# zju3dv/DetectorFreeSfM

Measured on NVIDIA B200. Metric: image-pairs/s coarse-match (hp2: tracks/s refinement), higher is better.
Workload: dtype f16x2-split (fp32-grade), fp32 accumulate

## Files before the change

### detectorfreesfm_b200/_lib.py

```python
import ctypes
import os

_HERE = os.path.dirname(os.path.abspath(__file__))
LIB_PATH = os.path.join(_HERE, "libdfsfm_b200.so")

_lib = None

c_void_p, c_int, c_float, c_char_p, c_int64 = ctypes.c_void_p, ctypes.c_int, ctypes.c_float, ctypes.c_char_p, ctypes.c_int64

PROTOTYPES = {
    "dfsfm_last_error": (c_char_p, []),
    "dfsfm_version": (c_int, []),
    "dfsfm_launch_count": (c_int64, []),
    "dfsfm_thread_set_pdl": (None, [c_int]),
    "dfsfm_debug_gemm_slab": (c_int, [c_void_p, c_int64, c_int, c_void_p, c_int64, c_int, c_void_p, c_int, c_int, c_int, c_void_p,
                                      c_int, c_int, c_void_p]),
    "dfsfm_set_engine": (None, [c_int]),
    "dfsfm_get_engine": (c_int, []),
    "dfsfm_profile_enable": (None, [c_int]),
    "dfsfm_profile_report": (c_int, [c_char_p, c_int]),
    "dfsfm_post_create": (c_int, [ctypes.POINTER(c_void_p), c_int]),
    "dfsfm_post_destroy": (None, [c_void_p]),
    "dfsfm_post_merge_keypoints": (c_int, [c_void_p, c_void_p, c_int64, c_int, c_void_p, c_void_p, c_int, c_void_p, c_void_p, c_void_p, c_void_p,
                                           ctypes.POINTER(c_int64), c_void_p]),
    "dfsfm_resize_lanczos_gray": (c_int, [c_void_p, c_int, c_int, c_int64, c_void_p, c_void_p, c_int, c_void_p, c_void_p, c_int, c_int, c_int,
                                          c_void_p, c_void_p, c_void_p]),
    "dfsfm_debug_timeline_arm": (c_int, [c_int]),
    "dfsfm_debug_timeline_read": (c_int, [c_void_p, c_void_p, c_int]),
    "dfsfm_coarse_create": (c_int, [ctypes.POINTER(c_void_p), c_int]),
    "dfsfm_coarse_destroy": (None, [c_void_p]),
    "dfsfm_coarse_set_param": (c_int, [c_void_p, c_char_p, c_void_p, c_int64, c_int64, c_int]),
    "dfsfm_coarse_features": (c_int, [c_void_p, c_void_p, c_int, c_int, c_void_p, c_void_p, c_void_p]),
    "dfsfm_coarse_features_fine": (c_int, [c_void_p, c_void_p, c_int, c_int, c_void_p, c_void_p, c_void_p, c_void_p]),
    "dfsfm_coarse_fine_match": (c_int, [c_void_p, c_void_p, c_int, c_int, c_void_p, c_int, c_int, c_void_p, c_int, c_void_p, c_int, c_void_p,
                                        c_void_p, c_int, c_void_p, c_void_p, c_void_p]),
    "dfsfm_coarse_transformer": (c_int, [c_void_p, c_void_p, c_int, c_void_p, c_int, c_void_p]),
    "dfsfm_coarse_match": (c_int, [c_void_p, c_void_p, c_int, c_int, c_void_p, c_int, c_int, c_float, c_int, c_float,
                                   c_void_p, c_void_p, c_void_p, c_void_p, c_int, c_void_p, c_void_p]),
    "dfsfm_crop_and_resize_forward": (c_int, [c_void_p, c_int, c_int, c_int, c_int, c_void_p, c_void_p, c_int, c_float,
                                              c_int, c_int, c_void_p, c_void_p]),
    "dfsfm_refine_create": (c_int, [ctypes.POINTER(c_void_p), c_int, c_int, c_int]),
    "dfsfm_refine_destroy": (None, [c_void_p]),
    "dfsfm_refine_set_param": (c_int, [c_void_p, c_char_p, c_void_p, c_int64, c_int64, c_int]),
    "dfsfm_refine_chunk": (c_int, [c_void_p, c_int, c_void_p, c_void_p, c_void_p, c_void_p, c_int, c_int, c_void_p, c_void_p,
                                   c_void_p, c_void_p, c_void_p, c_void_p, c_void_p, c_void_p, c_void_p, c_void_p]),
    "dfsfm_assign_bags": (c_int, [ctypes.POINTER(c_void_p), c_int64, c_void_p, c_void_p, c_void_p, c_void_p, c_int64, c_void_p, c_void_p, c_void_p,
                                  c_int, c_int, c_int]),
    "dfsfm_bags_sizes": (None, [c_void_p, ctypes.POINTER(c_int64), ctypes.POINTER(c_int64), ctypes.POINTER(c_int64), ctypes.POINTER(c_int64)]),
    "dfsfm_bags_export": (None, [c_void_p, c_void_p, c_void_p, c_void_p, c_void_p, c_void_p, c_void_p, c_void_p]),
    "dfsfm_bags_destroy": (None, [c_void_p]),
    "dfsfm_debug_pyset": (c_int, [c_int, c_void_p, c_int64, c_void_p, c_int64, c_void_p, ctypes.POINTER(c_int64)]),
    "dfsfm_debug_gemm": (c_int, [c_void_p, c_int64, c_int, c_void_p, c_int64, c_int, c_void_p, c_int, c_int, c_int, c_void_p,
                                 c_int, c_int, c_void_p]),
}


class DfsfmError(RuntimeError):
    pass


def load_library():
    global _lib
    if _lib is not None:
        return _lib
    if not os.path.exists(LIB_PATH):
# ... 25 lines not shown
```

### detectorfreesfm_b200/coarse_matcher.py

```python
import ctypes
from collections import OrderedDict

import torch

from . import _lib
from .packing import pack_loftr, position_encoding


class B200LoFTR(torch.nn.Module):
    def __init__(self, config, device=None, feature_cache_size=64, feature_cache_bytes=8 << 30):
        super().__init__()
        self.config = config
        mc = config["match_coarse"]
        if mc["match_type"] != "dual_softmax":
            raise NotImplementedError("only match_type='dual_softmax' is built (the shipped loftr_ds configs)")
        self.fine = bool(config["fine"]["enable"])
        if self.fine:
            fcfg = config["fine"]
            if (fcfg["d_model"] != 128 or fcfg["nhead"] != 8 or list(fcfg["layer_names"]) != ["self", "cross"] or config["fine_window_size"] != 5
                    or not config["fine_concat_coarse_feat"] or tuple(config["resolution"]) != (8, 2)):
                raise NotImplementedError("fine stage is specialised for the outdoor_ds LoFTR (window 5, d_model 128, ['self','cross'])")
        c = config["coarse"]
        if c["d_model"] != 256 or c["nhead"] != 8 or list(c["layer_names"]) != ["self", "cross"] * 4 or c["attention"] != "linear":
            raise NotImplementedError("engine is specialised for the outdoor_ds LoFTR (d_model 256, 8 heads, 8 layers, linear)")
# ... 32 lines not shown
        return self

    def load_state_dict(self, state_dict, strict=True):
        self._packed = pack_loftr(state_dict, fine=self.fine)
        if self._h:
            self._upload()
        self.clear_cache()
        return self

    def _upload(self):
        for name, (t, kind) in self._packed.items():
            _lib.check(self._lib.dfsfm_coarse_set_param(self._h, name.encode(), ctypes.c_void_p(t.data_ptr()), t.shape[0], t.shape[1], kind))

    def _destroy(self):
        if self._h:
            self._lib.dfsfm_coarse_destroy(self._h)
            self._h = ctypes.c_void_p()
        self._pe.clear()
        self._cache.clear()
        self._cache_bytes = 0

    def __del__(self):
        try:
            self._destroy()
        except Exception:
            pass

    def _pe_tokens(self, h, w):
        key = (h, w)
        if key not in self._pe:
            self._pe[key] = position_encoding(h, w).to(self._device)
        return self._pe[key]

    def extract_features(self, image, cache_key=None):
        assert image.is_cuda and image.dtype == torch.float32 and image.dim() == 4 and image.shape[0] == 1 and image.shape[1] == 1
        H, W = image.shape[2:]
        key = None if cache_key is None else (cache_key, H, W)
        if key is not None and key in self._cache:
            self._cache.move_to_end(key)
            return self._cache[key]
        image = image.contiguous()
        h, w = H // 8, W // 8
        tokens = torch.empty(h * w, 256, device=self._device, dtype=torch.float32)
        if self.fine:
            feat_f = torch.empty((H // 2) * (W // 2), 128, device=self._device, dtype=torch.float32)
            _lib.check(self._lib.dfsfm_coarse_features_fine(self._h, _lib.ptr(image), H, W, _lib.ptr(self._pe_tokens(h, w)), _lib.ptr(tokens),
                                                            _lib.ptr(feat_f), _lib.stream_ptr(self._device)))
            out = (tokens, feat_f)
        else:
            _lib.check(self._lib.dfsfm_coarse_features(self._h, _lib.ptr(image), H, W, _lib.ptr(self._pe_tokens(h, w)), _lib.ptr(tokens),
                                                       _lib.stream_ptr(self._device)))
            out = tokens
        if key is not None:
            nbytes = sum(t.numel() * t.element_size() for t in (out if isinstance(out, tuple) else (out,)))
            self._cache[key] = out
            self._cache_bytes += nbytes
            while len(self._cache) > 1 and (len(self._cache) > self._cache_size or self._cache_bytes > self._cache_bytes_max):
                _, old = self._cache.popitem(last=False)
                self._cache_bytes -= sum(t.numel() * t.element_size() for t in (old if isinstance(old, tuple) else (old,)))
        return out

    def fine_match(self, feat_f0, hw0_f, feat_f1, hw1_f, feat_c0, hw0_c, feat_c1, hw1_c, i_ids, j_ids):
        M = int(i_ids.shape[0])
        coords = torch.zeros(M, 2, device=self._device, dtype=torch.float32)
        std = torch.zeros(M, device=self._device, dtype=torch.float32)
        if M > 0:
            i32, j32 = i_ids.to(torch.int32).contiguous(), j_ids.to(torch.int32).contiguous()
            _lib.check(self._lib.dfsfm_coarse_fine_match(self._h, _lib.ptr(feat_f0), hw0_f[0], hw0_f[1], _lib.ptr(feat_f1), hw1_f[0], hw1_f[1],
                                                         _lib.ptr(feat_c0), hw0_c[1], _lib.ptr(feat_c1), hw1_c[1], _lib.ptr(i32), _lib.ptr(j32), M,
                                                         _lib.ptr(coords), _lib.ptr(std), _lib.stream_ptr(self._device)))
        return coords, std

    def transform(self, feat0, feat1):
        _lib.check(self._lib.dfsfm_coarse_transformer(self._h, _lib.ptr(feat0), feat0.shape[0], _lib.ptr(feat1), feat1.shape[0],
                                                      _lib.stream_ptr(self._device)))
        return feat0, feat1

    def coarse_match(self, feat0, hw0_c, feat1, hw1_c, return_conf=False):
        L, S = hw0_c[0] * hw0_c[1], hw1_c[0] * hw1_c[1]
        cap = min(L, S)
        i_ids = torch.empty(cap, device=self._device, dtype=torch.int32)
        j_ids = torch.empty(cap, device=self._device, dtype=torch.int32)
        mconf = torch.empty(cap, device=self._device, dtype=torch.float32)
        count = torch.zeros(1, device=self._device, dtype=torch.int32)
        conf = torch.empty(L, S, device=self._device, dtype=torch.float32) if return_conf else None
        _lib.check(self._lib.dfsfm_coarse_match(self._h, _lib.ptr(feat0), hw0_c[0], hw0_c[1], _lib.ptr(feat1), hw1_c[0], hw1_c[1],
                                                self.thr, self.border_rm, self.temperature, _lib.ptr(i_ids), _lib.ptr(j_ids),
                                                _lib.ptr(mconf), _lib.ptr(count), cap, _lib.ptr(conf), _lib.stream_ptr(self._device)))
        n = int(count.item())
        return i_ids[:n].long(), j_ids[:n].long(), mconf[:n], conf

    @torch.no_grad()
    def forward(self, data):
        if not self._h:
            raise _lib.DfsfmError("B200LoFTR: call .cuda() before forward (there is no CPU path)")
        with torch.cuda.device(self._device):
            return self._forward(data)

    def clear_cache(self):
        self._cache.clear()
        self._cache_bytes = 0

    def _forward(self, data):
        if not self._h:
            raise _lib.DfsfmError("B200LoFTR: call .cuda() before forward (there is no CPU path)")
        if self._packed is None:
            raise _lib.DfsfmError("B200LoFTR: load_state_dict() has not been called")
        im0, im1 = data["image0"], data["image1"]
        if im0.size(0) != 1:
            raise NotImplementedError("bs must be 1 (coarse_match_worker.py:86 asserts the same)")
        if "mask0" in data:
            raise NotImplementedError("padding masks are a training-time feature (loftr.py:61-63)")
        data.update({"bs": 1, "hw0_i": im0.shape[2:], "hw1_i": im1.shape[2:]})
        names = data.get("pair_key")
        k0 = k1 = None
        if names is not None:
            k0 = names[0][0] if isinstance(names[0], (list, tuple)) else names[0]
            k1 = names[1][0] if isinstance(names[1], (list, tuple)) else names[1]
        f0 = self.extract_features(im0, k0)
        f1 = self.extract_features(im1, k1)
        if self.fine:
            (f0, ff0), (f1, ff1) = f0, f1
        hw0_c = (im0.shape[2] // 8, im0.shape[3] // 8)
        hw1_c = (im1.shape[2] // 8, im1.shape[3] // 8)
        data.update({"hw0_c": torch.Size(hw0_c), "hw1_c": torch.Size(hw1_c)})
        f0, f1 = self.transform(f0.clone(), f1.clone())
        keep_conf = bool(data.get("_return_conf_matrix", False))
        i_ids, j_ids, mconf, conf = self.coarse_match(f0, hw0_c, f1, hw1_c, keep_conf)
        if keep_conf:
            data["conf_matrix"] = conf[None]
            data["feat_c0"], data["feat_c1"] = f0[None], f1[None]
        b_ids = torch.zeros_like(i_ids)
        scale = data["hw0_i"][0] / hw0_c[0]
        scale0 = scale * data["scale0"][b_ids][:, [1, 0]] if "scale0" in data else scale
        scale1 = scale * data["scale1"][b_ids][:, [1, 0]] if "scale1" in data else scale
        mkpts0_c = torch.stack([i_ids % hw0_c[1], i_ids // hw0_c[1]], dim=1) * scale0
        mkpts1_c = torch.stack([j_ids % hw1_c[1], j_ids // hw1_c[1]], dim=1) * scale1
        keep = mconf != 0
        data.update({
            "b_ids": b_ids, "i_ids": i_ids, "j_ids": j_ids, "gt_mask": mconf == 0,
            "m_bids": b_ids[keep], "mkpts0_c": mkpts0_c[keep], "mkpts1_c": mkpts1_c[keep], "mconf": mconf[keep],
        })
        if not self.fine:
            data.update({"mkpts0_f": data["mkpts0_c"], "mkpts1_f": data["mkpts1_c"]})
            return None
        hw0_f = (im0.shape[2] // 2, im0.shape[3] // 2)
        hw1_f = (im1.shape[2] // 2, im1.shape[3] // 2)
        data.update({"hw0_f": torch.Size(hw0_f), "hw1_f": torch.Size(hw1_f), "W": 5})
        coords2, std = self.fine_match(ff0, hw0_f, ff1, hw1_f, f0, hw0_c, f1, hw1_c, i_ids, j_ids)
        data["expec_f"] = torch.cat([coords2 / 2, std[:, None]], -1)
        scale_f = data["hw0_i"][0] / hw0_f[0]
        scale1_f = scale_f * data["scale1"][b_ids][:, [1, 0]] if "scale0" in data else scale_f
        data.update({"mkpts0_f": data["mkpts0_c"], "mkpts1_f": data["mkpts1_c"] + (coords2 * scale1_f)[:len(data["mconf"])]})
# ... 2 lines not shown
```

### detectorfreesfm_b200/csrc/coarse_engine.cu

```cuda
#include <algorithm>
#include <map>
#include <memory>

#include "../../include/dfsfm_b200.h"
#include "engine_common.h"
#include "fine_kernels.cuh"
#include "refine_kernels.cuh"

namespace dfsfm {

namespace {

struct Geom {
    int H, W, Hp, Wp;
    long long rows;
    Geom() : H(0), W(0), Hp(0), Wp(0), rows(0) {}
    Geom(int h, int w) : H(h), W(w), Hp(h + 1), Wp(w + 1), rows(static_cast<long long>(h + 1) * (w + 1)) {}
    FlatGeom flat() const { return FlatGeom{Hp, Wp, H, W}; }
};

struct ParityBuf {
    __half* base = nullptr;
    long long rows = 0;
    int C = 0;
    HL plane(int k) const {
        HL b;
        b.hi = base + static_cast<long long>(k) * 2 * rows * C;
        b.rows = rows;
        b.C = C;
        return b;
    }
    long long plane_stride() const { return 2 * rows * C; }
};

struct FeatWs {
// ... 19 lines not shown
struct TokWs {
    int cap = 0;
    HL x[2], msg[2], m1[2], hid[2];
    float* qkv[2] = {nullptr, nullptr};
    float* xf = nullptr;
    HL g;
    float* ksum = nullptr;
    float* kvp_part = nullptr;
    unsigned* kvp_flags = nullptr;
    int L = 0, L1 = 0, S = 0;
    int kv_chunks = 0;
    float* kv_part = nullptr;
    float* kv_state = nullptr;
    Seg* seg_dev = nullptr;
    float2* part = nullptr;
    float* stat[2] = {nullptr, nullptr};
    unsigned long long* best[2] = {nullptr, nullptr};
};

}

class CoarseEngine {
  public:
    explicit CoarseEngine(int device) : device_(device) {
        DFSFM_CUDA(cudaSetDevice(device));
        DFSFM_CUDA(cudaFuncSetAttribute(attn_apply_kernel<32>, cudaFuncAttributeMaxDynamicSharedMemorySize, attn_smem_bytes<32>()));
    }
    ~CoarseEngine() {
        for (auto& kv : feat_ws_) free_feat(kv.second);
        free_tok(tok_);
    }
    ParamStore params;

    void features(const float* img, int H, int W, const float* pe, float* tokens, float* feat_f, cudaStream_t st);
    void fine_match(const float* ff0, int Hf0, int Wf0, const float* ff1, int Hf1, int Wf1, const float* fc0, int w0c, const float* fc1, int w1c,
                    const int* i_ids, const int* j_ids, int M, float* coords_out, float* std_out, cudaStream_t st);
    void transformer(float* f0, int L, float* f1, int S, cudaStream_t st);
    void match(const float* f0, int h0c, int w0c, const float* f1, int h1c, int w1c, float thr, int border, float temperature, int* i_ids,
               int* j_ids, float* mconf, int* n_matches, int capacity, float* conf_out, cudaStream_t st);

  private:
    int device_;
    std::map<std::pair<int, int>, FeatWs> feat_ws_;
    TokWs tok_;
    unsigned kv_epoch_ = 0;
    FineWs fine_;
    void ensure_fine(int M);
    void fine_branch(FeatWs& w, float* feat_f, cudaStream_t st);
    void layer128(int li, bool self, int x0, int xn, int s0, int sn, const Seg* kv_segs, int n_kv, const Seg* apply_segs, int n_apply, cudaStream_t st);

    FeatWs& get_feat_ws(int H, int W);
    void ensure_tok(int n);
    static void free_feat(FeatWs& w);
    static void free_tok(TokWs& w);

    template <int BN>
    void conv(const HL* ins, int n_in, GemmCore core, const std::string& wname, ConvEpiParams ep, cudaStream_t st);
    void layer_call(int li, bool self, int x0, int xn, int s0, int sn, int kv_seg0, int n_segs, int apply_seg0, int max_count, cudaStream_t st,
                    int seg_row0 = 0);
};

static int kv_tok() {
    static int v = 0;
    if (!v) {
        const char* e = getenv("DFSFM_KV_TOK");
        v = e ? atoi(e) : kKvTokPerCta;
        if (v < 16) v = 16;
    }
    return v;
}
static bool attn_fold() {
    static int v = -1;
    if (v < 0) {
        const char* e = getenv("DFSFM_ATTN_FOLD");
        v = (e && e[0] == '0') ? 0 : 1;
    }
    return v == 1 && engine_version() == 2;
}
static bool kv_epi() {
    static int v = -1;
    if (v < 0) {
        const char* e = getenv("DFSFM_KV_EPI");
        v = (e && e[0] == '0') ? 0 : 1;
    }
    return v == 1;
}
static bool enc_fused() {
    static int v = -1;
    if (v < 0) {
        const char* e = getenv("DFSFM_ENC_FUSED");
        v = (e && e[0] == '0') ? 0 : 1;
    }
    return v == 1;
}
static bool lin_bn128() {
    static int v = -1;
    if (v < 0) {
        const char* e = getenv("DFSFM_LIN_BN128");
        v = (e && e[0] == '1') ? 1 : 0;
    }
    return v == 1;
}

static ParityBuf parity_alloc(long long rows, int C) {
    ParityBuf p;
    p.rows = rows;
    p.C = C;
    const size_t bytes = static_cast<size_t>(8) * rows * C * sizeof(__half);
    DFSFM_CUDA(cudaMalloc(&p.base, bytes));
    zero_device_sync(p.base, 0, bytes);
    return p;
}

FeatWs& CoarseEngine::get_feat_ws(int H, int W) {
    auto key = std::make_pair(H, W);
    auto it = feat_ws_.find(key);
    if (it != feat_ws_.end()) return it->second;
    if (feat_ws_.size() >= 8) {
        for (auto& kv : feat_ws_) free_feat(kv.second);
        feat_ws_.clear();
    }
    FeatWs w;
    w.g2 = Geom(H / 2, W / 2);
    w.g4 = Geom(H / 4, W / 4);
    w.g8 = Geom(H / 8, W / 8);
    w.a2 = hl_alloc(w.g2.rows, 128);
    w.b2 = hl_alloc(w.g2.rows, 128);
    w.c2 = hl_alloc(w.g2.rows, 128);
    w.p1 = parity_alloc(w.g4.rows, 128);
    w.a4 = hl_alloc(w.g4.rows, 208);
    w.b4 = hl_alloc(w.g4.rows, 208);
    w.p2 = parity_alloc(w.g8.rows, 208);
    w.a8 = hl_alloc(w.g8.rows, 256);
    w.b8 = hl_alloc(w.g8.rows, 256);
    w.c8 = hl_alloc(w.g8.rows, 256);
    return feat_ws_.emplace(key, w).first->second;
}
void CoarseEngine::free_feat(FeatWs& w) {
    hl_free(w.a2); hl_free(w.b2); hl_free(w.c2); hl_free(w.a4); hl_free(w.b4); hl_free(w.a8); hl_free(w.b8); hl_free(w.c8);
    if (w.p1.base) cudaFree(w.p1.base);
    if (w.p2.base) cudaFree(w.p2.base);
    if (w.fine) {
        hl_free(w.x3o); hl_free(w.t4a); hl_free(w.t4b); hl_free(w.x2o); hl_free(w.t2a); hl_free(w.t2b);
        cudaFree(w.f4); cudaFree(w.f2);
    }
}

template <int BN>
void CoarseEngine::conv(const HL* ins, int n_in, GemmCore core, const std::string& wname, ConvEpiParams ep, cudaStream_t st) {
    const HL& w = params.mat(wname + ".w");
    const bool slab = BN <= 128 && slab_applicable(core, n_in);
    TmapPack maps;
    for (int i = 0; i < kMaxAMaps; ++i) maps.a[i] = make_tmap(ins[i < n_in ? i : 0], slab ? kSlabRows : kBM);
    maps.b = make_tmap(w, bbox(BN));
    core.b_row0 = 0;
    DFSFM_CHECK(static_cast<long long>(core.num_taps) * core.cpad == w.C, "weight K does not match taps*cpad for " + wname);
    ep.M = core.M;
    ep.bias = params.has_vec(wname + ".b") ? params.vec(wname + ".b") : nullptr;
    if constexpr (BN <= 128) {
        if (slab) {
            launch_gemm_slab_counted<BN, ConvEpi>(maps, core, ep, ep.N, st, "conv");
            return;
        }
    }
    launch_gemm_counted<BN, true, ConvEpi>(maps, core, ep, ep.N, st, "conv");
}

static ConvEpiParams epi_flat(const Geom& g, int N, const HL& out, bool relu, const HL* res) {
    ConvEpiParams e;
    memset(&e, 0, sizeof(e));
    e.N = N;
    e.g = g.flat();
    e.relu = relu ? 1 : 0;
    if (res) { e.res_hi = res->hi; e.res_lo = res->lo(); e.res_ld = res->C; }
    e.out_mode = OUT_FLAT;
    e.out_hi = out.hi;
    e.out_lo = out.lo();
    e.out_ld = out.C;
    return e;
}
static ConvEpiParams epi_parity(const Geom& g, int N, const ParityBuf& out, bool relu, const HL* res) {
    ConvEpiParams e = epi_flat(g, N, out.plane(0), relu, res);
    e.out_mode = OUT_PARITY;
    e.plane_stride = out.plane_stride();
    return e;
}

void CoarseEngine::features(const float* img, int H, int W, const float* pe, float* tokens, float* feat_f, cudaStream_t st) {
    DFSFM_CHECK(H % 8 == 0 && W % 8 == 0 && H >= 16 && W >= 16, "image size must be a multiple of 8 (CoarseMatchingDataset df=8)");
    FeatWs& w = get_feat_ws(H, W);
    {
        dim3 grid((w.g2.W + kStemTW - 1) / kStemTW, (w.g2.H + kStemTH - 1) / kStemTH, 1);
        { LaunchScope ls("stem", st);
          stem_conv_kernel<<<grid, 128, 0, st>>>(img, H, W, params.vec("stem.w"), params.vec("stem.b"), w.a2.hi, w.a2.lo()); }
        DFSFM_CUDA(cudaGetLastError());
    }
    GemmCore c;
    memset(&c, 0, sizeof(c));
    c.M = static_cast<int>(w.g2.rows);
    set_k(c, 128);
    conv_taps_s1(c, 3, w.g2.Wp);
    { const HL in[1] = {w.a2}; conv<128>(in, 1, c, "l1.0.c1", epi_flat(w.g2, 128, w.b2, true, nullptr), st); }
    { const HL in[1] = {w.b2}; conv<128>(in, 1, c, "l1.0.c2", epi_flat(w.g2, 128, w.c2, true, &w.a2), st); }
    { const HL in[1] = {w.c2}; conv<128>(in, 1, c, "l1.1.c1", epi_flat(w.g2, 128, w.b2, true, nullptr), st); }
    { const HL in[1] = {w.b2}; conv<128>(in, 1, c, "l1.1.c2", epi_parity(w.g2, 128, w.p1, true, &w.c2), st); }
    c.M = static_cast<int>(w.g4.rows);
    set_k(c, 128);
    conv_taps_s2(c, w.g4.Wp);
    { const HL in[4] = {w.p1.plane(0), w.p1.plane(1), w.p1.plane(2), w.p1.plane(3)};
      conv<208>(in, 4, c, "l2.0.c1", epi_flat(w.g4, 208, w.a4, true, nullptr), st); }
    set_k(c, 208);
    conv_taps_s1(c, 3, w.g4.Wp);
    c.num_taps = 10; c.tap_map[9] = 1; c.tap_shift[9] = 0;
    { const HL in[2] = {w.a4, w.p1.plane(0)}; conv<208>(in, 2, c, "l2.0.c2", epi_flat(w.g4, 208, w.b4, true, nullptr), st); }
    conv_taps_s1(c, 3, w.g4.Wp);
    { const HL in[1] = {w.b4}; conv<208>(in, 1, c, "l2.1.c1", epi_flat(w.g4, 208, w.a4, true, nullptr), st); }
    { const HL in[1] = {w.a4}; conv<208>(in, 1, c, "l2.1.c2", epi_parity(w.g4, 208, w.p2, true, &w.b4), st); }
    c.M = static_cast<int>(w.g8.rows);
    set_k(c, 208);
    conv_taps_s2(c, w.g8.Wp);
    { const HL in[4] = {w.p2.plane(0), w.p2.plane(1), w.p2.plane(2), w.p2.plane(3)};
      conv<256>(in, 4, c, "l3.0.c1", epi_flat(w.g8, 256, w.a8, true, nullptr), st); }
    set_k(c, 256);
    conv_taps_s1(c, 3, w.g8.Wp);
    c.num_taps = 10; c.tap_map[9] = 1; c.tap_shift[9] = 0;
    { const HL in[2] = {w.a8, w.p2.plane(0)}; conv<256>(in, 2, c, "l3.0.c2", epi_flat(w.g8, 256, w.b8, true, nullptr), st); }
    conv_taps_s1(c, 3, w.g8.Wp);
    { const HL in[1] = {w.b8}; conv<256>(in, 1, c, "l3.1.c1", epi_flat(w.g8, 256, w.a8, true, nullptr), st); }
    { const HL in[1] = {w.a8}; conv<256>(in, 1, c, "l3.1.c2", epi_flat(w.g8, 256, w.c8, true, &w.b8), st); }
    conv_taps_s1(c, 1, w.g8.Wp);
    {
        ConvEpiParams e;
        memset(&e, 0, sizeof(e));
        e.N = 256;
        e.g = w.g8.flat();
        e.addend = pe;
        e.out_mode = OUT_DENSE;
        e.out_f32 = tokens;
        e.out_f32_ld = 256;
        if (feat_f) {
            if (!w.fine) {
                w.x3o = hl_alloc(w.g8.rows, 256);
                w.t4a = hl_alloc(w.g4.rows, 256); w.t4b = hl_alloc(w.g4.rows, 256); w.x2o = hl_alloc(w.g4.rows, 208);
                w.t2a = hl_alloc(w.g2.rows, 208); w.t2b = hl_alloc(w.g2.rows, 208);
                DFSFM_CUDA(cudaMalloc(&w.f4, static_cast<size_t>(w.g4.rows) * 256 * sizeof(float)));
                DFSFM_CUDA(cudaMalloc(&w.f2, static_cast<size_t>(w.g2.rows) * 208 * sizeof(float)));
                w.fine = true;
            }
        }
        const HL in[1] = {w.c8};
        conv<256>(in, 1, c, "out3", e, st);
        if (feat_f) {
            ConvEpiParams e2 = epi_flat(w.g8, 256, w.x3o, false, nullptr);
            conv<256>(in, 1, c, "out3", e2, st);
            fine_branch(w, feat_f, st);
        }
    }
}

void CoarseEngine::fine_branch(FeatWs& w, float* feat_f, cudaStream_t st) {
    GemmCore c;
    memset(&c, 0, sizeof(c));
    auto up_add = [&](const HL& low, const Geom& gl, int C, const float* lateral, const HL& out) {
        const long long total = static_cast<long long>(2 * gl.H) * (2 * gl.W) * (C / 8);
        LaunchScope ls("upsample", st);
        upsample2x_add_kernel<<<static_cast<unsigned>((total + 255) / 256), 256, 0, st>>>(low.hi, low.lo(), gl.H, gl.W, C, lateral, out.hi, out.lo(), total);
        DFSFM_CUDA(cudaGetLastError());
    };
    c.M = static_cast<int>(w.g8.rows);
    set_k(c, 208);
    conv_taps_s1(c, 1, w.g8.Wp);
    for (int k = 0; k < 4; ++k) {
        ConvEpiParams e;
        memset(&e, 0, sizeof(e));
        e.N = 256; e.g = w.g8.flat(); e.out_mode = OUT_UNPARITY; e.upy = k >> 1; e.upx = k & 1; e.ohp = w.g4.Hp; e.owp = w.g4.Wp;
        e.out_f32 = w.f4; e.out_f32_ld = 256;
        const HL in[1] = {w.p2.plane(k)};
        conv<256>(in, 1, c, "fpn.l2o", e, st);
    }
    up_add(w.x3o, w.g8, 256, w.f4, w.t4a);
    c.M = static_cast<int>(w.g4.rows);
    set_k(c, 256);
    conv_taps_s1(c, 3, w.g4.Wp);
    { ConvEpiParams e = epi_flat(w.g4, 256, w.t4b, false, nullptr); e.relu = 2; const HL in[1] = {w.t4a}; conv<256>(in, 1, c, "fpn.l2o2a", e, st); }
    { ConvEpiParams e = epi_flat(w.g4, 208, w.x2o, false, nullptr); const HL in[1] = {w.t4b}; conv<208>(in, 1, c, "fpn.l2o2b", e, st); }
    set_k(c, 128);
    conv_taps_s1(c, 1, w.g4.Wp);
// ... 516 lines not shown
    }
    layer128(0, true, 0, R, 0, R, f.segs, 2 * M, f.segs, 2 * M, st);
    layer128(1, false, 0, MW, MW, MW, f.segs + M, M, f.segs + 2 * M, M, st);
    layer128(1, false, MW, MW, 0, MW, f.segs, M, f.segs + 3 * M, M, st);
    {
        const size_t smem = fine_match_smem_bytes(5, 1);
        DFSFM_CUDA(cudaMemsetAsync(coords_out, 0, static_cast<size_t>(M) * 2 * sizeof(float), st));
        LaunchScope ls("fine_match", st);
        fine_match_kernel<<<M, kFmThreads, smem, st>>>(f.xf, f.tracks, f.views, 1, 5, 1, f.d_query, coords_out, std_out, M);
        DFSFM_CUDA(cudaGetLastError());
    }
}

}

using dfsfm::CoarseEngine;
struct dfsfm_coarse { std::unique_ptr<CoarseEngine> e; };

extern "C" {

int dfsfm_coarse_create(dfsfm_coarse_t** out, int device) {
    return dfsfm::guard([&] {
        auto* h = new dfsfm_coarse;
        h->e.reset(new CoarseEngine(device));
        *out = h;
    });
}
void dfsfm_coarse_destroy(dfsfm_coarse_t* h) { delete h; }

int dfsfm_coarse_set_param(dfsfm_coarse_t* h, const char* name, const float* host, int64_t rows, int64_t cols, int kind) {
    return dfsfm::guard([&] { h->e->params.set(name, host, rows, cols, kind); });
}
int dfsfm_coarse_features(dfsfm_coarse_t* h, const float* image_dev, int H, int W, const float* pe_dev, float* tokens_out_dev, void* stream) {
    return dfsfm::guard([&] { h->e->features(image_dev, H, W, pe_dev, tokens_out_dev, nullptr, static_cast<cudaStream_t>(stream)); });
}
int dfsfm_coarse_features_fine(dfsfm_coarse_t* h, const float* image_dev, int H, int W, const float* pe_dev, float* tokens_out_dev,
                               float* feat_f_out_dev, void* stream) {
    return dfsfm::guard([&] { h->e->features(image_dev, H, W, pe_dev, tokens_out_dev, feat_f_out_dev, static_cast<cudaStream_t>(stream)); });
}
int dfsfm_coarse_fine_match(dfsfm_coarse_t* h, const float* feat_f0_dev, int Hf0, int Wf0, const float* feat_f1_dev, int Hf1, int Wf1,
                            const float* feat_c0_dev, int w0c, const float* feat_c1_dev, int w1c, const int32_t* i_ids_dev,
                            const int32_t* j_ids_dev, int M, float* coords_out_dev, float* std_out_dev, void* stream) {
    return dfsfm::guard([&] {
        h->e->fine_match(feat_f0_dev, Hf0, Wf0, feat_f1_dev, Hf1, Wf1, feat_c0_dev, w0c, feat_c1_dev, w1c, i_ids_dev, j_ids_dev, M, coords_out_dev,
                         std_out_dev, static_cast<cudaStream_t>(stream));
    });
}
int dfsfm_coarse_transformer(dfsfm_coarse_t* h, float* feat0_dev, int L, float* feat1_dev, int S, void* stream) {
    return dfsfm::guard([&] { h->e->transformer(feat0_dev, L, feat1_dev, S, static_cast<cudaStream_t>(stream)); });
}
int dfsfm_coarse_match(dfsfm_coarse_t* h, const float* feat0_dev, int h0c, int w0c, const float* feat1_dev, int h1c, int w1c, float thr,
                       int border_rm, float temperature, int32_t* i_ids_dev, int32_t* j_ids_dev, float* mconf_dev, int32_t* n_matches_dev,
                       int capacity, float* conf_out_dev, void* stream) {
    return dfsfm::guard([&] {
        h->e->match(feat0_dev, h0c, w0c, feat1_dev, h1c, w1c, thr, border_rm, temperature, i_ids_dev, j_ids_dev, mconf_dev, n_matches_dev,
                    capacity, conf_out_dev, static_cast<cudaStream_t>(stream));
    });
}

}
```

### detectorfreesfm_b200/csrc/gemm_engine.cuh

```cuda
#pragma once
#include "tc_common.cuh"

namespace dfsfm {

constexpr int kBM = 128;
constexpr int kBK = 64;
constexpr int kMaxTaps = 26;
constexpr int kMaxAMaps = 5;
constexpr int kGemmThreads = 192;
constexpr int kGemm2EpiWarps = 8;
constexpr int kGemm2Threads = 64 + 32 * kGemm2EpiWarps;

struct EpiCtx {
    uint8_t* stg;
    uint8_t* stg_partner;
    int bar_id;
};

struct TmapPack {
    CUtensorMap a[kMaxAMaps];
    CUtensorMap b;
};

struct GemmCore {
// ... 410 lines not shown
        tmem_ld_wait();
    }
}

struct FlatGeom {
    int Hp, Wp, H, W;
};

enum OutMode : int {
    OUT_FLAT = 0,
    OUT_PARITY = 1,
    OUT_DENSE = 2,
    OUT_WINDOW = 3,
    OUT_WINDOW_DENSE = 4,
    OUT_UNPARITY = 5,
};

struct ConvEpiParams {
    int M, N;
    FlatGeom g;
    const float* bias;
    int relu;
    const __half* res_hi;
    const __half* res_lo;
    int res_ld;
    const float* addend;
    int addend_mode;
    int out_mode;
    __half* out_hi;
    __half* out_lo;
    int out_ld;
    long long plane_stride;
    float* out_f32;
    int out_f32_ld;
    int wy0, wx0, wh, ww;
    int ohp, owp;
    int upy, upx;
};

struct ConvEpi {
    using Params = ConvEpiParams;
    static constexpr bool kHasState = false;
    static constexpr bool kSeparateCorr = true;
    static constexpr int kEpiStageBytes = 0;
    template <int BN, int kCorr>
    static __device__ __forceinline__ void run(const Params& p, uint32_t tmem_warp, int row0, int lane, int n0, int cb, int ce, int part_idx, const EpiCtx& ctx) {
        const int row = row0 + lane;
        bool valid = row < p.M;
        int n_img = 0, y = 0, x = 0;
        if (p.g.Hp > 0) {
            const int per = p.g.Hp * p.g.Wp;
            n_img = row / per;
            const int r = row - n_img * per;
            y = r / p.g.Wp;
            x = r - y * p.g.Wp;
            valid = valid && (y < p.g.H) && (x < p.g.W);
        }
        long long orow = row;
        long long obase = 0;
        if (p.out_mode == OUT_PARITY) {
            const int Hp2 = p.g.H / 2 + 1, Wp2 = p.g.W / 2 + 1;
            obase = static_cast<long long>((y & 1) * 2 + (x & 1)) * p.plane_stride;
            orow = static_cast<long long>(n_img) * Hp2 * Wp2 + (y >> 1) * Wp2 + (x >> 1);
        } else if (p.out_mode == OUT_DENSE) {
            orow = static_cast<long long>(n_img) * p.g.H * p.g.W + y * p.g.W + x;
        } else if (p.out_mode == OUT_WINDOW) {
            valid = valid && y >= p.wy0 && y < p.wy0 + p.wh && x >= p.wx0 && x < p.wx0 + p.ww;
            orow = static_cast<long long>(n_img) * p.ohp * p.owp + (y - p.wy0) * p.owp + (x - p.wx0);
        } else if (p.out_mode == OUT_WINDOW_DENSE) {
            valid = valid && y >= p.wy0 && y < p.wy0 + p.wh && x >= p.wx0 && x < p.wx0 + p.ww;
            orow = static_cast<long long>(n_img) * p.wh * p.ww + (y - p.wy0) * p.ww + (x - p.wx0);
        } else if (p.out_mode == OUT_UNPARITY) {
            orow = static_cast<long long>(n_img) * p.ohp * p.owp + (2 * y + p.upy) * p.owp + (2 * x + p.upx);
        }
#pragma unroll 1
        for (int c0 = cb; c0 < ce; c0 += 32) {
            float v[32];
            load_acc32<kCorr>(tmem_warp + c0, v);
            const int nb = n0 + c0;
            if (!valid || nb >= p.N) continue;
            const int ncnt = p.N - nb;
            if (p.bias) {
#pragma unroll
                for (int j = 0; j < 32; j += 4) {
                    if (j < ncnt) {
                        const float4 b4 = __ldg(reinterpret_cast<const float4*>(p.bias + nb + j));
                        v[j] += b4.x; v[j + 1] += b4.y; v[j + 2] += b4.z; v[j + 3] += b4.w;
                    }
                }
            }
            if (p.res_hi) {
                const __half* rh = p.res_hi + static_cast<long long>(row) * p.res_ld + nb;
                const __half* rl = p.res_lo + static_cast<long long>(row) * p.res_ld + nb;
#pragma unroll
                for (int j = 0; j < 32; j += 8) {
                    if (j < ncnt) {
                        const uint4 uh = *reinterpret_cast<const uint4*>(rh + j);
                        const uint4 ul = *reinterpret_cast<const uint4*>(rl + j);
// ... 22 lines not shown
            if (p.relu == 1) {
#pragma unroll
                for (int j = 0; j < 32; ++j) v[j] = fmaxf(v[j], 0.f);
            } else if (p.relu == 2) {
#pragma unroll
                for (int j = 0; j < 32; ++j) v[j] = v[j] > 0.f ? v[j] : 0.01f * v[j];
            }
            if (p.out_hi) {
                __half* oh = p.out_hi + obase + orow * p.out_ld + nb;
                __half* ol = p.out_lo ? p.out_lo + obase + orow * p.out_ld + nb : nullptr;
#pragma unroll
                for (int j = 0; j < 32; j += 8) {
                    if (j < ncnt) {
                        uint4 uh, ul;
                        __half* hh = reinterpret_cast<__half*>(&uh);
                        __half* hl = reinterpret_cast<__half*>(&ul);
#pragma unroll
                        for (int q = 0; q < 8; ++q) split_f16(v[j + q], hh[q], hl[q]);
                        *reinterpret_cast<uint4*>(oh + j) = uh;
                        if (ol) *reinterpret_cast<uint4*>(ol + j) = ul;
                    }
                }
            }
            if (p.addend && p.addend_mode == 0) {
                const float* ad = p.addend + static_cast<long long>(y * p.g.W + x) * p.N + nb;
#pragma unroll
                for (int j = 0; j < 32; j += 4) {
                    if (j < ncnt) {
                        const float4 a4 = __ldg(reinterpret_cast<const float4*>(ad + j));
                        v[j] += a4.x; v[j + 1] += a4.y; v[j + 2] += a4.z; v[j + 3] += a4.w;
                    }
                }
            }
            if (p.out_f32) {
                float* of = p.out_f32 + orow * p.out_f32_ld + nb;
#pragma unroll
                for (int j = 0; j < 32; j += 4) {
                    if (j < ncnt) *reinterpret_cast<float4*>(of + j) = make_float4(v[j], v[j + 1], v[j + 2], v[j + 3]);
                }
            }
        }
    }
};


enum LinMode : int {
    LIN_F32_ELU = 0,
    LIN_RELU_HL = 1,
    LIN_LN = 2,
    LIN_QZ = 3,
};

struct LinEpiParams {
    int M, N;
    int mode;
    int elu_cols;
    const float* gamma;
    const float* beta;
    const float* resid;
    int resid_ld;
    const __half* res_hi;
    const __half* res_lo;
    int res_ld;
    float* out_f32;
    int out_f32_ld;
    int out_col0;
    const float* ksum;
    int seg_row0;
// ... 508 lines not shown
```

### detectorfreesfm_b200/csrc/simt_kernels.cuh

```cuda
#pragma once
#include "tc_common.cuh"

namespace dfsfm {

constexpr int kStemTH = 8, kStemTW = 16;
static __global__ void __launch_bounds__(128) stem_conv_kernel(const float* __restrict__ img, int H, int W, const float* __restrict__ w ,
                                                        const float* __restrict__ bias, __half* __restrict__ out_hi,
                                                        __half* __restrict__ out_lo) {
    constexpr int IH = kStemTH * 2 + 5, IW = kStemTW * 2 + 5;
    constexpr int PITCH = 40;
    __shared__ __align__(16) float tile[IH][PITCH];
    const int H2 = H / 2, W2 = W / 2, Wp = W2 + 1;
    const int oy0 = blockIdx.y * kStemTH, ox0 = blockIdx.x * kStemTW;
    const int n = blockIdx.z;
    const float* im = img + static_cast<long long>(n) * H * W;
    for (int i = threadIdx.x; i < IH * PITCH; i += 128) {
        const int ty = i / PITCH, tx = i - ty * PITCH;
        const int iy = oy0 * 2 - 3 + ty, ix = ox0 * 2 - 3 + tx;
        tile[ty][tx] = (tx < IW && iy >= 0 && iy < H && ix >= 0 && ix < W) ? im[static_cast<long long>(iy) * W + ix] : 0.f;
    }
    const int c = threadIdx.x;
    float wr[49];
#pragma unroll
    for (int i = 0; i < 49; ++i) wr[i] = w[c * 49 + i];
    const float b = bias[c];
    __syncthreads();
    const long long img_rows = static_cast<long long>(H2 + 1) * Wp;
    for (int py = 0; py < kStemTH; ++py) {
        const int oy = oy0 + py;
        if (oy >= H2) break;
#pragma unroll 1
        for (int pg = 0; pg < kStemTW / 4; ++pg) {
            float acc[4] = {0.f, 0.f, 0.f, 0.f};
#pragma unroll
            for (int ky = 0; ky < 7; ++ky) {
                float in[16];
                const float4* rp = reinterpret_cast<const float4*>(&tile[py * 2 + ky][pg * 8]);
#pragma unroll
                for (int q = 0; q < 4; ++q) {
                    const float4 v = rp[q];
                    in[4 * q] = v.x; in[4 * q + 1] = v.y; in[4 * q + 2] = v.z; in[4 * q + 3] = v.w;
                }
#pragma unroll
                for (int p = 0; p < 4; ++p)
#pragma unroll
                    for (int kx = 0; kx < 7; ++kx) acc[p] = fmaf(wr[ky * 7 + kx], in[2 * p + kx], acc[p]);
            }
#pragma unroll
// ... 400 lines not shown
```

### include/dfsfm_b200.h

```cpp
#ifndef DFSFM_B200_H_
#define DFSFM_B200_H_

#include <stdint.h>

#ifdef __cplusplus
extern "C" {
#endif

const char* dfsfm_last_error(void);
int dfsfm_version(void);

typedef struct dfsfm_coarse dfsfm_coarse_t;

int dfsfm_coarse_create(dfsfm_coarse_t** out, int device);
void dfsfm_coarse_destroy(dfsfm_coarse_t* h);

int dfsfm_coarse_set_param(dfsfm_coarse_t* h, const char* name, const float* host, int64_t rows, int64_t cols, int kind);

int dfsfm_coarse_features(dfsfm_coarse_t* h, const float* image_dev, int H, int W, const float* pe_dev, float* tokens_out_dev,
                          void* stream);

int dfsfm_coarse_features_fine(dfsfm_coarse_t* h, const float* image_dev, int H, int W, const float* pe_dev, float* tokens_out_dev,
                               float* feat_f_out_dev, void* stream);

int dfsfm_coarse_fine_match(dfsfm_coarse_t* h, const float* feat_f0_dev, int Hf0, int Wf0, const float* feat_f1_dev, int Hf1, int Wf1,
                            const float* feat_c0_dev, int w0c, const float* feat_c1_dev, int w1c, const int32_t* i_ids_dev,
                            const int32_t* j_ids_dev, int M, float* coords_out_dev, float* std_out_dev, void* stream);

int dfsfm_coarse_transformer(dfsfm_coarse_t* h, float* feat0_dev, int L, float* feat1_dev, int S, void* stream);

int dfsfm_coarse_match(dfsfm_coarse_t* h, const float* feat0_dev, int h0c, int w0c, const float* feat1_dev, int h1c, int w1c, float thr,
                       int border_rm, float temperature, int32_t* i_ids_dev, int32_t* j_ids_dev, float* mconf_dev,
                       int32_t* n_matches_dev, int capacity, float* conf_out_dev, void* stream);

int dfsfm_crop_and_resize_forward(const float* image_dev, int batch, int depth, int image_h, int image_w, const float* boxes_dev,
                                  const int32_t* box_index_dev, int num_boxes, float extrapolation_value, int crop_h, int crop_w,
                                  float* crops_dev, void* stream);

typedef struct dfsfm_refine dfsfm_refine_t;

int dfsfm_refine_create(dfsfm_refine_t** out, int device, int window, int left_window);
void dfsfm_refine_destroy(dfsfm_refine_t* h);
int dfsfm_refine_set_param(dfsfm_refine_t* h, const char* name, const float* host, int64_t rows, int64_t cols, int kind);

int dfsfm_refine_chunk(dfsfm_refine_t* h, int n_img, const float* const* images_dev, const int32_t* H, const int32_t* W,
                       const float* scales_hw, int M, int Nq, const float* query_pts, const float* ref_pts, const uint8_t* valid,
                       const int32_t* q_img_idx, const int32_t* r_img_idx, const uint8_t* movable, float* query_refined,
                       float* ref_refined, float* std_out, void* stream);

typedef struct dfsfm_post dfsfm_post_t;
int dfsfm_post_create(dfsfm_post_t** out, int device);
void dfsfm_post_destroy(dfsfm_post_t* h);
int dfsfm_post_merge_keypoints(dfsfm_post_t* h, const float* rows_dev, int64_t n_rows, int n_pairs, const int64_t* pair_offset_dev,
// ... 35 lines not shown
```

Before: 212.6.

## Batch both images of a pair through one CNN backbone pass

```diff
diff --git a/detectorfreesfm_b200/_lib.py b/detectorfreesfm_b200/_lib.py
--- a/detectorfreesfm_b200/_lib.py
+++ b/detectorfreesfm_b200/_lib.py
@@ -31,6 +31,7 @@
     "dfsfm_coarse_destroy": (None, [c_void_p]),
     "dfsfm_coarse_set_param": (c_int, [c_void_p, c_char_p, c_void_p, c_int64, c_int64, c_int]),
     "dfsfm_coarse_features": (c_int, [c_void_p, c_void_p, c_int, c_int, c_void_p, c_void_p, c_void_p]),
+    "dfsfm_coarse_features_pair": (c_int, [c_void_p, c_void_p, c_void_p, c_int, c_int, c_void_p, c_void_p, c_void_p, c_void_p]),
     "dfsfm_coarse_features_fine": (c_int, [c_void_p, c_void_p, c_int, c_int, c_void_p, c_void_p, c_void_p, c_void_p]),
     "dfsfm_coarse_fine_match": (c_int, [c_void_p, c_void_p, c_int, c_int, c_void_p, c_int, c_int, c_void_p, c_int, c_void_p, c_int, c_void_p,
                                         c_void_p, c_int, c_void_p, c_void_p, c_void_p]),
diff --git a/detectorfreesfm_b200/coarse_matcher.py b/detectorfreesfm_b200/coarse_matcher.py
--- a/detectorfreesfm_b200/coarse_matcher.py
+++ b/detectorfreesfm_b200/coarse_matcher.py
@@ -88,13 +88,17 @@
             self._pe[key] = position_encoding(h, w).to(self._device)
         return self._pe[key]
 
+    @staticmethod
+    def _cache_key(image, cache_key):
+        assert image.is_cuda and image.dtype == torch.float32 and image.dim() == 4 and image.shape[0] == 1 and image.shape[1] == 1
+        return None if cache_key is None else (cache_key, image.shape[2], image.shape[3])
+
     def extract_features(self, image, cache_key=None):
-        assert image.is_cuda and image.dtype == torch.float32 and image.dim() == 4 and image.shape[0] == 1 and image.shape[1] == 1
-        H, W = image.shape[2:]
-        key = None if cache_key is None else (cache_key, H, W)
+        key = self._cache_key(image, cache_key)
         if key is not None and key in self._cache:
             self._cache.move_to_end(key)
             return self._cache[key]
+        H, W = image.shape[2:]
         image = image.contiguous()
         h, w = H // 8, W // 8
         tokens = torch.empty(h * w, 256, device=self._device, dtype=torch.float32)
@@ -107,14 +111,36 @@
             _lib.check(self._lib.dfsfm_coarse_features(self._h, _lib.ptr(image), H, W, _lib.ptr(self._pe_tokens(h, w)), _lib.ptr(tokens),
                                                        _lib.stream_ptr(self._device)))
             out = tokens
-        if key is not None:
-            nbytes = sum(t.numel() * t.element_size() for t in (out if isinstance(out, tuple) else (out,)))
-            self._cache[key] = out
-            self._cache_bytes += nbytes
-            while len(self._cache) > 1 and (len(self._cache) > self._cache_size or self._cache_bytes > self._cache_bytes_max):
-                _, old = self._cache.popitem(last=False)
-                self._cache_bytes -= sum(t.numel() * t.element_size() for t in (old if isinstance(old, tuple) else (old,)))
+        self._cache_put(key, out)
         return out
+
+    def extract_features_pair(self, image0, image1, cache_key0=None, cache_key1=None):
+        key0, key1 = self._cache_key(image0, cache_key0), self._cache_key(image1, cache_key1)
+        assert self._pair_applies(image0, image1, key0, key1)
+        H, W = image0.shape[2:]
+        image0, image1 = image0.contiguous(), image1.contiguous()
+        h, w = H // 8, W // 8
+        tokens0 = torch.empty(h * w, 256, device=self._device, dtype=torch.float32)
+        tokens1 = torch.empty(h * w, 256, device=self._device, dtype=torch.float32)
+        _lib.check(self._lib.dfsfm_coarse_features_pair(self._h, _lib.ptr(image0), _lib.ptr(image1), H, W, _lib.ptr(self._pe_tokens(h, w)),
+                                                        _lib.ptr(tokens0), _lib.ptr(tokens1), _lib.stream_ptr(self._device)))
+        self._cache_put(key0, tokens0)
+        self._cache_put(key1, tokens1)
+        return tokens0, tokens1
+
+    def _pair_applies(self, image0, image1, key0, key1):
+        return (not self.fine and image0.shape == image1.shape and (key0 is None or (key0 not in self._cache and key0 != key1))
+                and (key1 is None or key1 not in self._cache))
+
+    def _cache_put(self, key, out):
+        if key is None:
+            return
+        nbytes = sum(t.numel() * t.element_size() for t in (out if isinstance(out, tuple) else (out,)))
+        self._cache[key] = out
+        self._cache_bytes += nbytes
+        while len(self._cache) > 1 and (len(self._cache) > self._cache_size or self._cache_bytes > self._cache_bytes_max):
+            _, old = self._cache.popitem(last=False)
+            self._cache_bytes -= sum(t.numel() * t.element_size() for t in (old if isinstance(old, tuple) else (old,)))
 
     def fine_match(self, feat_f0, hw0_f, feat_f1, hw1_f, feat_c0, hw0_c, feat_c1, hw1_c, i_ids, j_ids):
         M = int(i_ids.shape[0])
@@ -173,8 +199,11 @@
         if names is not None:
             k0 = names[0][0] if isinstance(names[0], (list, tuple)) else names[0]
             k1 = names[1][0] if isinstance(names[1], (list, tuple)) else names[1]
-        f0 = self.extract_features(im0, k0)
-        f1 = self.extract_features(im1, k1)
+        if self._pair_applies(im0, im1, self._cache_key(im0, k0), self._cache_key(im1, k1)):
+            f0, f1 = self.extract_features_pair(im0, im1, k0, k1)
+        else:
+            f0 = self.extract_features(im0, k0)
+            f1 = self.extract_features(im1, k1)
         if self.fine:
             (f0, ff0), (f1, ff1) = f0, f1
         hw0_c = (im0.shape[2] // 8, im0.shape[3] // 8)
diff --git a/detectorfreesfm_b200/csrc/coarse_engine.cu b/detectorfreesfm_b200/csrc/coarse_engine.cu
--- a/detectorfreesfm_b200/csrc/coarse_engine.cu
+++ b/detectorfreesfm_b200/csrc/coarse_engine.cu
@@ -1,6 +1,7 @@
 #include <algorithm>
 #include <map>
 #include <memory>
+#include <tuple>
 
 #include "../../include/dfsfm_b200.h"
 #include "engine_common.h"
@@ -86,7 +87,7 @@
     }
     ParamStore params;
 
-    void features(const float* img, int H, int W, const float* pe, float* tokens, float* feat_f, cudaStream_t st);
+    void features(const float* const* imgs, int n_img, int H, int W, const float* pe, float* const* tokens, float* feat_f, cudaStream_t st);
     void fine_match(const float* ff0, int Hf0, int Wf0, const float* ff1, int Hf1, int Wf1, const float* fc0, int w0c, const float* fc1, int w1c,
                     const int* i_ids, const int* j_ids, int M, float* coords_out, float* std_out, cudaStream_t st);
     void transformer(float* f0, int L, float* f1, int S, cudaStream_t st);
@@ -95,7 +96,7 @@
 
   private:
     int device_;
-    std::map<std::pair<int, int>, FeatWs> feat_ws_;
+    std::map<std::tuple<int, int, int>, FeatWs> feat_ws_;
     TokWs tok_;
     unsigned kv_epoch_ = 0;
     FineWs fine_;
@@ -103,13 +104,14 @@
     void fine_branch(FeatWs& w, float* feat_f, cudaStream_t st);
     void layer128(int li, bool self, int x0, int xn, int s0, int sn, const Seg* kv_segs, int n_kv, const Seg* apply_segs, int n_apply, cudaStream_t st);
 
-    FeatWs& get_feat_ws(int H, int W);
+    FeatWs& get_feat_ws(int H, int W, int n_img);
     void ensure_tok(int n);
     static void free_feat(FeatWs& w);
     static void free_tok(TokWs& w);
 
     template <int BN>
-    void conv(const HL* ins, int n_in, GemmCore core, const std::string& wname, ConvEpiParams ep, cudaStream_t st);
+    void conv(const HL* ins, int n_in, GemmCore core, const std::string& wname, ConvEpiParams ep, cudaStream_t st, bool allow_slab = true);
+    void conv_l3(int bn, const HL* ins, int n_in, const GemmCore& core, const std::string& wname, const ConvEpiParams& ep, cudaStream_t st);
     void layer_call(int li, bool self, int x0, int xn, int s0, int sn, int kv_seg0, int n_segs, int apply_seg0, int max_count, cudaStream_t st,
                     int seg_row0 = 0);
 };
@@ -166,8 +168,8 @@
     return p;
 }
 
-FeatWs& CoarseEngine::get_feat_ws(int H, int W) {
-    auto key = std::make_pair(H, W);
+FeatWs& CoarseEngine::get_feat_ws(int H, int W, int n_img) {
+    const auto key = std::make_tuple(H, W, n_img);
     auto it = feat_ws_.find(key);
     if (it != feat_ws_.end()) return it->second;
     if (feat_ws_.size() >= 8) {
@@ -178,16 +180,17 @@
     w.g2 = Geom(H / 2, W / 2);
     w.g4 = Geom(H / 4, W / 4);
     w.g8 = Geom(H / 8, W / 8);
-    w.a2 = hl_alloc(w.g2.rows, 128);
-    w.b2 = hl_alloc(w.g2.rows, 128);
-    w.c2 = hl_alloc(w.g2.rows, 128);
-    w.p1 = parity_alloc(w.g4.rows, 128);
-    w.a4 = hl_alloc(w.g4.rows, 208);
-    w.b4 = hl_alloc(w.g4.rows, 208);
-    w.p2 = parity_alloc(w.g8.rows, 208);
-    w.a8 = hl_alloc(w.g8.rows, 256);
-    w.b8 = hl_alloc(w.g8.rows, 256);
-    w.c8 = hl_alloc(w.g8.rows, 256);
+    DFSFM_CHECK(n_img * w.g2.rows < (1ll << 31), "image too large for 32-bit row indices");
+    w.a2 = hl_alloc(n_img * w.g2.rows, 128);
+    w.b2 = hl_alloc(n_img * w.g2.rows, 128);
+    w.c2 = hl_alloc(n_img * w.g2.rows, 128);
+    w.p1 = parity_alloc(n_img * w.g4.rows, 128);
+    w.a4 = hl_alloc(n_img * w.g4.rows, 208);
+    w.b4 = hl_alloc(n_img * w.g4.rows, 208);
+    w.p2 = parity_alloc(n_img * w.g8.rows, 208);
+    w.a8 = hl_alloc(n_img * w.g8.rows, 256);
+    w.b8 = hl_alloc(n_img * w.g8.rows, 256);
+    w.c8 = hl_alloc(n_img * w.g8.rows, 256);
     return feat_ws_.emplace(key, w).first->second;
 }
 void CoarseEngine::free_feat(FeatWs& w) {
@@ -201,9 +204,9 @@
 }
 
 template <int BN>
-void CoarseEngine::conv(const HL* ins, int n_in, GemmCore core, const std::string& wname, ConvEpiParams ep, cudaStream_t st) {
+void CoarseEngine::conv(const HL* ins, int n_in, GemmCore core, const std::string& wname, ConvEpiParams ep, cudaStream_t st, bool allow_slab) {
     const HL& w = params.mat(wname + ".w");
-    const bool slab = BN <= 128 && slab_applicable(core, n_in);
+    const bool slab = BN <= 128 && allow_slab && slab_applicable(core, n_in);
     TmapPack maps;
     for (int i = 0; i < kMaxAMaps; ++i) maps.a[i] = make_tmap(ins[i < n_in ? i : 0], slab ? kSlabRows : kBM);
     maps.b = make_tmap(w, bbox(BN));
@@ -218,6 +221,19 @@
         }
     }
     launch_gemm_counted<BN, true, ConvEpi>(maps, core, ep, ep.N, st, "conv");
+}
+
+static int layer3_bn(int M) {
+    const int pairs = sm_count() / 2;
+    const int row_tiles = (M + 2 * kBM - 1) / (2 * kBM);
+    const int full_rounds = (row_tiles + pairs - 1) / pairs;
+    const int half_rounds = (2 * row_tiles + pairs - 1) / pairs;
+    return half_rounds < 2 * full_rounds ? 128 : 256;
+}
+void CoarseEngine::conv_l3(int bn, const HL* ins, int n_in, const GemmCore& core, const std::string& wname, const ConvEpiParams& ep,
+                           cudaStream_t st) {
+    if (bn == 128) conv<128>(ins, n_in, core, wname, ep, st, false);
+    else conv<256>(ins, n_in, core, wname, ep, st);
 }
 
 static ConvEpiParams epi_flat(const Geom& g, int N, const HL& out, bool relu, const HL* res) {
@@ -240,25 +256,27 @@
     return e;
 }
 
-void CoarseEngine::features(const float* img, int H, int W, const float* pe, float* tokens, float* feat_f, cudaStream_t st) {
+void CoarseEngine::features(const float* const* imgs, int n_img, int H, int W, const float* pe, float* const* tokens, float* feat_f,
+                            cudaStream_t st) {
     DFSFM_CHECK(H % 8 == 0 && W % 8 == 0 && H >= 16 && W >= 16, "image size must be a multiple of 8 (CoarseMatchingDataset df=8)");
-    FeatWs& w = get_feat_ws(H, W);
-    {
-        dim3 grid((w.g2.W + kStemTW - 1) / kStemTW, (w.g2.H + kStemTH - 1) / kStemTH, 1);
+    DFSFM_CHECK(n_img == 1 || (n_img == 2 && !feat_f), "one image, or two without the fine branch");
+    FeatWs& w = get_feat_ws(H, W, n_img);
+    {
+        dim3 grid((w.g2.W + kStemTW - 1) / kStemTW, (w.g2.H + kStemTH - 1) / kStemTH, n_img);
         { LaunchScope ls("stem", st);
-          stem_conv_kernel<<<grid, 128, 0, st>>>(img, H, W, params.vec("stem.w"), params.vec("stem.b"), w.a2.hi, w.a2.lo()); }
+          stem_conv_kernel<<<grid, 128, 0, st>>>(imgs[0], imgs[n_img - 1], H, W, params.vec("stem.w"), params.vec("stem.b"), w.a2.hi, w.a2.lo()); }
         DFSFM_CUDA(cudaGetLastError());
     }
     GemmCore c;
     memset(&c, 0, sizeof(c));
-    c.M = static_cast<int>(w.g2.rows);
+    c.M = static_cast<int>(n_img * w.g2.rows);
     set_k(c, 128);
     conv_taps_s1(c, 3, w.g2.Wp);
     { const HL in[1] = {w.a2}; conv<128>(in, 1, c, "l1.0.c1", epi_flat(w.g2, 128, w.b2, true, nullptr), st); }
     { const HL in[1] = {w.b2}; conv<128>(in, 1, c, "l1.0.c2", epi_flat(w.g2, 128, w.c2, true, &w.a2), st); }
     { const HL in[1] = {w.c2}; conv<128>(in, 1, c, "l1.1.c1", epi_flat(w.g2, 128, w.b2, true, nullptr), st); }
     { const HL in[1] = {w.b2}; conv<128>(in, 1, c, "l1.1.c2", epi_parity(w.g2, 128, w.p1, true, &w.c2), st); }
-    c.M = static_cast<int>(w.g4.rows);
+    c.M = static_cast<int>(n_img * w.g4.rows);
     set_k(c, 128);
     conv_taps_s2(c, w.g4.Wp);
     { const HL in[4] = {w.p1.plane(0), w.p1.plane(1), w.p1.plane(2), w.p1.plane(3)};
@@ -270,18 +288,19 @@
     conv_taps_s1(c, 3, w.g4.Wp);
     { const HL in[1] = {w.b4}; conv<208>(in, 1, c, "l2.1.c1", epi_flat(w.g4, 208, w.a4, true, nullptr), st); }
     { const HL in[1] = {w.a4}; conv<208>(in, 1, c, "l2.1.c2", epi_parity(w.g4, 208, w.p2, true, &w.b4), st); }
-    c.M = static_cast<int>(w.g8.rows);
+    c.M = static_cast<int>(n_img * w.g8.rows);
+    const int bn3 = layer3_bn(c.M);
     set_k(c, 208);
     conv_taps_s2(c, w.g8.Wp);
     { const HL in[4] = {w.p2.plane(0), w.p2.plane(1), w.p2.plane(2), w.p2.plane(3)};
-      conv<256>(in, 4, c, "l3.0.c1", epi_flat(w.g8, 256, w.a8, true, nullptr), st); }
+      conv_l3(bn3, in, 4, c, "l3.0.c1", epi_flat(w.g8, 256, w.a8, true, nullptr), st); }
     set_k(c, 256);
     conv_taps_s1(c, 3, w.g8.Wp);
     c.num_taps = 10; c.tap_map[9] = 1; c.tap_shift[9] = 0;
-    { const HL in[2] = {w.a8, w.p2.plane(0)}; conv<256>(in, 2, c, "l3.0.c2", epi_flat(w.g8, 256, w.b8, true, nullptr), st); }
+    { const HL in[2] = {w.a8, w.p2.plane(0)}; conv_l3(bn3, in, 2, c, "l3.0.c2", epi_flat(w.g8, 256, w.b8, true, nullptr), st); }
     conv_taps_s1(c, 3, w.g8.Wp);
-    { const HL in[1] = {w.b8}; conv<256>(in, 1, c, "l3.1.c1", epi_flat(w.g8, 256, w.a8, true, nullptr), st); }
-    { const HL in[1] = {w.a8}; conv<256>(in, 1, c, "l3.1.c2", epi_flat(w.g8, 256, w.c8, true, &w.b8), st); }
+    { const HL in[1] = {w.b8}; conv_l3(bn3, in, 1, c, "l3.1.c1", epi_flat(w.g8, 256, w.a8, true, nullptr), st); }
+    { const HL in[1] = {w.a8}; conv_l3(bn3, in, 1, c, "l3.1.c2", epi_flat(w.g8, 256, w.c8, true, &w.b8), st); }
     conv_taps_s1(c, 1, w.g8.Wp);
     {
         ConvEpiParams e;
@@ -290,7 +309,8 @@
         e.g = w.g8.flat();
         e.addend = pe;
         e.out_mode = OUT_DENSE;
-        e.out_f32 = tokens;
+        e.out_f32 = tokens[0];
+        e.out_f32_1 = n_img == 2 ? tokens[1] : nullptr;
         e.out_f32_ld = 256;
         if (feat_f) {
             if (!w.fine) {
@@ -303,10 +323,10 @@
             }
         }
         const HL in[1] = {w.c8};
-        conv<256>(in, 1, c, "out3", e, st);
+        conv_l3(bn3, in, 1, c, "out3", e, st);
         if (feat_f) {
             ConvEpiParams e2 = epi_flat(w.g8, 256, w.x3o, false, nullptr);
-            conv<256>(in, 1, c, "out3", e2, st);
+            conv_l3(bn3, in, 1, c, "out3", e2, st);
             fine_branch(w, feat_f, st);
         }
     }
@@ -889,11 +909,19 @@
     return dfsfm::guard([&] { h->e->params.set(name, host, rows, cols, kind); });
 }
 int dfsfm_coarse_features(dfsfm_coarse_t* h, const float* image_dev, int H, int W, const float* pe_dev, float* tokens_out_dev, void* stream) {
-    return dfsfm::guard([&] { h->e->features(image_dev, H, W, pe_dev, tokens_out_dev, nullptr, static_cast<cudaStream_t>(stream)); });
+    return dfsfm::guard([&] { h->e->features(&image_dev, 1, H, W, pe_dev, &tokens_out_dev, nullptr, static_cast<cudaStream_t>(stream)); });
+}
+int dfsfm_coarse_features_pair(dfsfm_coarse_t* h, const float* image0_dev, const float* image1_dev, int H, int W, const float* pe_dev,
+                               float* tokens0_out_dev, float* tokens1_out_dev, void* stream) {
+    return dfsfm::guard([&] {
+        const float* imgs[2] = {image0_dev, image1_dev};
+        float* tokens[2] = {tokens0_out_dev, tokens1_out_dev};
+        h->e->features(imgs, 2, H, W, pe_dev, tokens, nullptr, static_cast<cudaStream_t>(stream));
+    });
 }
 int dfsfm_coarse_features_fine(dfsfm_coarse_t* h, const float* image_dev, int H, int W, const float* pe_dev, float* tokens_out_dev,
                                float* feat_f_out_dev, void* stream) {
-    return dfsfm::guard([&] { h->e->features(image_dev, H, W, pe_dev, tokens_out_dev, feat_f_out_dev, static_cast<cudaStream_t>(stream)); });
+    return dfsfm::guard([&] { h->e->features(&image_dev, 1, H, W, pe_dev, &tokens_out_dev, feat_f_out_dev, static_cast<cudaStream_t>(stream)); });
 }
 int dfsfm_coarse_fine_match(dfsfm_coarse_t* h, const float* feat_f0_dev, int Hf0, int Wf0, const float* feat_f1_dev, int Hf1, int Wf1,
                             const float* feat_c0_dev, int w0c, const float* feat_c1_dev, int w1c, const int32_t* i_ids_dev,
diff --git a/detectorfreesfm_b200/csrc/gemm_engine.cuh b/detectorfreesfm_b200/csrc/gemm_engine.cuh
--- a/detectorfreesfm_b200/csrc/gemm_engine.cuh
+++ b/detectorfreesfm_b200/csrc/gemm_engine.cuh
@@ -466,6 +466,7 @@
     int out_ld;
     long long plane_stride;
     float* out_f32;
+    float* out_f32_1;
     int out_f32_ld;
     int wy0, wx0, wh, ww;
     int ohp, owp;
@@ -492,12 +493,18 @@
         }
         long long orow = row;
         long long obase = 0;
+        float* out_f32 = p.out_f32;
         if (p.out_mode == OUT_PARITY) {
             const int Hp2 = p.g.H / 2 + 1, Wp2 = p.g.W / 2 + 1;
             obase = static_cast<long long>((y & 1) * 2 + (x & 1)) * p.plane_stride;
             orow = static_cast<long long>(n_img) * Hp2 * Wp2 + (y >> 1) * Wp2 + (x >> 1);
         } else if (p.out_mode == OUT_DENSE) {
-            orow = static_cast<long long>(n_img) * p.g.H * p.g.W + y * p.g.W + x;
+            if (n_img == 1 && p.out_f32_1) {
+                out_f32 = p.out_f32_1;
+                orow = y * p.g.W + x;
+            } else {
+                orow = static_cast<long long>(n_img) * p.g.H * p.g.W + y * p.g.W + x;
+            }
         } else if (p.out_mode == OUT_WINDOW) {
             valid = valid && y >= p.wy0 && y < p.wy0 + p.wh && x >= p.wx0 && x < p.wx0 + p.ww;
             orow = static_cast<long long>(n_img) * p.ohp * p.owp + (y - p.wy0) * p.owp + (x - p.wx0);
@@ -586,8 +593,8 @@
                     }
                 }
             }
-            if (p.out_f32) {
-                float* of = p.out_f32 + orow * p.out_f32_ld + nb;
+            if (out_f32) {
+                float* of = out_f32 + orow * p.out_f32_ld + nb;
 #pragma unroll
                 for (int j = 0; j < 32; j += 4) {
                     if (j < ncnt) *reinterpret_cast<float4*>(of + j) = make_float4(v[j], v[j + 1], v[j + 2], v[j + 3]);
diff --git a/detectorfreesfm_b200/csrc/simt_kernels.cuh b/detectorfreesfm_b200/csrc/simt_kernels.cuh
--- a/detectorfreesfm_b200/csrc/simt_kernels.cuh
+++ b/detectorfreesfm_b200/csrc/simt_kernels.cuh
@@ -4,16 +4,16 @@
 namespace dfsfm {
 
 constexpr int kStemTH = 8, kStemTW = 16;
-static __global__ void __launch_bounds__(128) stem_conv_kernel(const float* __restrict__ img, int H, int W, const float* __restrict__ w ,
-                                                        const float* __restrict__ bias, __half* __restrict__ out_hi,
-                                                        __half* __restrict__ out_lo) {
+static __global__ void __launch_bounds__(128) stem_conv_kernel(const float* __restrict__ img0, const float* __restrict__ img1, int H, int W,
+                                                        const float* __restrict__ w , const float* __restrict__ bias,
+                                                        __half* __restrict__ out_hi, __half* __restrict__ out_lo) {
     constexpr int IH = kStemTH * 2 + 5, IW = kStemTW * 2 + 5;
     constexpr int PITCH = 40;
     __shared__ __align__(16) float tile[IH][PITCH];
     const int H2 = H / 2, W2 = W / 2, Wp = W2 + 1;
     const int oy0 = blockIdx.y * kStemTH, ox0 = blockIdx.x * kStemTW;
     const int n = blockIdx.z;
-    const float* im = img + static_cast<long long>(n) * H * W;
+    const float* im = n == 0 ? img0 : img1;
     for (int i = threadIdx.x; i < IH * PITCH; i += 128) {
         const int ty = i / PITCH, tx = i - ty * PITCH;
         const int iy = oy0 * 2 - 3 + ty, ix = ox0 * 2 - 3 + tx;
diff --git a/include/dfsfm_b200.h b/include/dfsfm_b200.h
--- a/include/dfsfm_b200.h
+++ b/include/dfsfm_b200.h
@@ -19,6 +19,9 @@
 
 int dfsfm_coarse_features(dfsfm_coarse_t* h, const float* image_dev, int H, int W, const float* pe_dev, float* tokens_out_dev,
                           void* stream);
+
+int dfsfm_coarse_features_pair(dfsfm_coarse_t* h, const float* image0_dev, const float* image1_dev, int H, int W, const float* pe_dev,
+                               float* tokens0_out_dev, float* tokens1_out_dev, void* stream);
 
 int dfsfm_coarse_features_fine(dfsfm_coarse_t* h, const float* image_dev, int H, int W, const float* pe_dev, float* tokens_out_dev,
                                float* feat_f_out_dev, void* stream);
```

Result: faster. 227.5 (median of 6 runs) (+7.0%).
